# francescoolivieri/Gymnast_OptimalControl

Hardware: AMD Instinct MI355X
Metric: swing-up Newton iterations/sec (batch×T states/s) at 1/2/4/8 MI355X (higher is better)
Workload: dtype f64

## Files before the change

gymnast_optimalcontrol_amd/_lib.py:

```python
from __future__ import annotations

import ctypes as C
import os

import torch

from . import _build

LIB_PATH = os.environ.get("GYM_LIB_PATH") or _build.LIB_PATH

EXPORTS = (
    "gym_abi_version", "gym_build_id", "gym_model_from_params",
    "gym_continuous_dynamics", "gym_rk4_step", "gym_jacobians", "gym_stage_cost_derivs",
    "gym_pack_lanes", "gym_unpack_lanes", "gym_unpack_gains",
    "gym_rollout_open_loop", "gym_closed_loop", "gym_total_cost", "gym_backward_sweep", "gym_linearize",
    "gym_riccati_general",
    "gym_newton_init", "gym_newton_init_warm", "gym_newton_iteration", "gym_newton_pipeline_split", "gym_newton_phase", "gym_newton_phase_kind",
    "gym_newton_run",
    "gym_newton_tail", "gym_newton_tail_scratch", "gym_newton_cand_scratch", "gym_newton_tail_lds",
    "gym_newton_finalize", "gym_newton_fill_states", "gym_placement_probe", "gym_newton_sigma",
    "gym_gamma_sweep", "gym_newton_gamma_sweep",
    "gym_tv_lqr_gains", "gym_dare_fixed_point", "gym_mpc_gains", "gym_lq_forward", "gym_track_rollout", "gym_track_rollout_ex",
    "gym_mpc_gains_all", "gym_mpc_box_workspace", "gym_mpc_box_qp", "gym_mpc_box_rollout",
    "gym_lqr_lanes_workspace", "gym_lqr_lanes_gains", "gym_lqr_lanes_rollout",
    "gym_mpc_lanes_gains",
    "gym_mpc_box_lanes_workspace", "gym_mpc_box_lanes_rollout",
    "gym_timing_create", "gym_timing_destroy", "gym_timing_collect",
)
KERNEL_KINDS = ("backward", "trial", "candidates", "retry", "stats", "phase_odd", "phase_even", "sigma", "run",
                "tail")

ABI_VERSION = 18
MAX_BP = 1 << 26
MPC_MAX_STAGES = 256
FLAG_U0_ZERO = 1
FLAG_X_CKPT = 2
FLAG_RUN_SINGLE = 4
FLAG_REF_LANE = 8
FLAG_SIGMA_STREAM = 16
TRACK_SINGLE = 1
CKPT_INTERVAL = 4

ACTIVE, CONVERGED, LS_FAILED, MAX_ITERS, PAD = 0, 1, 2, 3, 4
STATUS_NAMES = {ACTIVE: "active", CONVERGED: "converged", LS_FAILED: "ls_failed", MAX_ITERS: "max_iters", PAD: "pad"}


class GymModel(C.Structure):
    _fields_ = [(n, C.c_double) for n in ("a", "b", "d", "g1", "g2", "f1", "f2", "dt")]


class GymWeights(C.Structure):
    _fields_ = [("Q", C.c_double * 4), ("R", C.c_double * 2), ("QT", C.c_double * 4)]


class GymArmijo(C.Structure):
    _fields_ = [("tol", C.c_double), ("beta", C.c_double), ("c", C.c_double), ("gamma0", C.c_double),
                ("max_ls", C.c_int32), ("record_history", C.c_int32)]


_P = C.c_void_p


TIMING_POOL = 512


class GymTiming(C.Structure):
    _fields_ = [("ev", _P * 20), ("ms", C.c_double * 10), ("launches", C.c_int64 * 10), ("pending", C.c_int32),
                ("pool_used", C.c_int32), ("pool_ev", _P * (2 * TIMING_POOL)), ("pool_kind", C.c_int32 * TIMING_POOL)]


class GymBatch(C.Structure):
    _fields_ = [("B", C.c_int64), ("Bp", C.c_int64), ("N", C.c_int32), ("hist_len", C.c_int32),
                ("flags", C.c_int32), ("pad", C.c_int32), ("x", _P * 2), ("u", _P * 2), ("K1", _P), ("cs", _P), ("x_ref", _P), ("u_ref", _P),
                ("cost", _P), ("dJ", _P), ("smax", _P), ("gamma", _P), ("status", _P), ("n_iter", _P),
                ("res_buf", _P), ("n_roll", _P), ("retry_list", _P), ("counters", _P), ("cand_ok", _P),
                ("partials", _P), ("stats", _P), ("hist_cost", _P), ("hist_smax", _P), ("lane_map", _P),
                ("timing", C.POINTER(GymTiming)), ("cand_scratch", _P), ("cand_slots", C.c_int64)]


_I64, _I32, _D = C.c_int64, C.c_int32, C.c_double
_MP, _WP, _AP, _BP = C.POINTER(GymModel), C.POINTER(GymWeights), C.POINTER(GymArmijo), C.POINTER(GymBatch)
_SIGS = {
    "gym_abi_version": [],
    "gym_model_from_params": [_P, _D, _MP],
    "gym_continuous_dynamics": [_MP, _P, _P, _P, _I64, _P],
    "gym_rk4_step": [_MP, _P, _P, _P, _I64, _P],
    "gym_jacobians": [_MP, _P, _P, _P, _P, _I64, _P],
    "gym_stage_cost_derivs": [_P, _P, _P, _P, _P, _P, _I32, _P, _P, _P, _I64, _P],
    "gym_pack_lanes": [_P, _P, _I64, _I64, _I32, _I32, _I32, _P],
    "gym_unpack_lanes": [_P, _P, _P, _P, _I64, _I64, _I32, _I32, _I32, _P],
    "gym_unpack_gains": [_P, _P, _I64, _I64, _I32, _P],
    "gym_rollout_open_loop": [_MP, _WP, _P, _P, _P, _P, _P, _P, _I64, _I64, _I32, _P],
    "gym_closed_loop": [_MP, _WP, _P, _P, _P, _P, _P, _P, _P, _P, _P, _P, _I64, _I64, _I32, _P],
    "gym_total_cost": [_P, _P, _P, _P, _P, _P, _P, _P, _I64, _I64, _I32, _P],
    "gym_backward_sweep": [_MP, _WP, _P, _P, _P, _P, _P, _P, _P, _P, _P, _I64, _I64, _I32, _P],
    "gym_linearize": [_MP, _WP, _P, _P, _P, _P, _P, _P, _P, _P, _P, _I64, _I64, _I32, _P],
    "gym_riccati_general": [_P] * 12 + [_I64, _I64, _I32, _P],
    "gym_newton_init": [_MP, _WP, _P, _BP, _P],
    "gym_newton_init_warm": [_MP, _WP, _P, _P, _P, _BP, _P],
    "gym_newton_iteration": [_MP, _WP, _AP, _BP, _I32, _P],
    "gym_newton_pipeline_split": [_BP, C.POINTER(C.c_int64)],
    "gym_newton_phase_kind": [_BP, C.POINTER(C.c_int32)],
    "gym_newton_phase": [_MP, _WP, _AP, _BP, _I32, _I32, _P],
    "gym_newton_run": [_MP, _WP, _AP, _BP, _I32, _I32, _P],
    "gym_newton_tail": [_MP, _WP, _AP, _BP, _P, _I32, _P, _I64, _I32, _I32, _P],
    "gym_newton_tail_scratch": [_I32, _I32, _I32, C.POINTER(C.c_int64)],
    "gym_newton_cand_scratch": [_I32, _I64, C.POINTER(C.c_int64)],
    "gym_newton_tail_lds": [_I32, C.POINTER(C.c_int64), C.POINTER(C.c_int64)],
    "gym_newton_finalize": [_MP, _WP, _BP, _I32, _P, _P, _P, _P, _P],
    "gym_newton_fill_states": [_MP, _BP, _I32, _P],
    "gym_placement_probe": [_BP, _I32, _P],
    "gym_newton_sigma": [_MP, _WP, _BP, _P, _P],
    "gym_gamma_sweep": [_MP, _WP, _P, _P, _P, _P, _P, _I32, _P, _P, _P, _I64, _I64, _I32, _P],
    "gym_newton_gamma_sweep": [_MP, _WP, _AP, _BP, _I32, _P, _I32, _P, _P],
    "gym_tv_lqr_gains": [_P, _P, _I32, _P, _P, _P, _P, _P, _I32, _I32, _I32, _I32, _D, _P, _P],
    "gym_dare_fixed_point": [_P, _P, _P, _P, _I32, _D, _P, _P, _P],
    "gym_mpc_gains": [_MP, _P, _P, _I32, _P, _P, _P, _P, _I32, _I32, _I32, _D, _P, _P, _P, _P],
    "gym_lq_forward": [_P, _P, _I32, _P, _P, _I32, _D, _P, _P, _I32, _P, _P, _P],
    "gym_track_rollout": [_MP, _P, _P, _P, _P, _I64, _I32, _P, _P, _P],
    "gym_track_rollout_ex": [_MP, _P, _P, _P, _P, _I64, _I32, _I32, _P, _P, _P],
    "gym_mpc_gains_all": [_MP, _P, _P, _I32, _P, _P, _P, _P, _I32, _I32, _I32, _D, _P, _P, _P, _P],
    "gym_mpc_box_workspace": [_I64, _I32, _I32, C.POINTER(C.c_int64)],
    "gym_mpc_box_qp": [_P, _P, _P, _I32, _P, _P, _P, _P, _I64, _I32, _D, _I32, _P, _I64, _P, _P, _P, _P, _P],
    "gym_mpc_box_rollout": [_MP, _P, _P, _P, _P, _P, _P, _P, _P, _P, _I64, _I32, _I32, _D, _I32, _P, _I64, _P, _P, _P,
                            _P, _P],
    "gym_lqr_lanes_workspace": [_I64, _I32, C.POINTER(C.c_int64)],
    "gym_lqr_lanes_gains": [_MP, _P, _P, _I64, _I32, _P, _P, _P, _P, _I64, _P, _P],
    "gym_lqr_lanes_rollout": [_MP, _P, _I64, _I32, _I32, _P, _I64, _P, _P, _P, _P],
    "gym_mpc_lanes_gains": [_MP, _P, _P, _I64, _I32, _I32, _P, _P, _P, _P, _I64, _P, _P],
    "gym_mpc_box_lanes_workspace": [_I64, _I32, _I32, C.POINTER(C.c_int64)],
    "gym_mpc_box_lanes_rollout": [_MP, _P, _P, _P, _I64, _I32, _I32, _I32, _P, _P, _P, _D, _I32, _P, _I64, _P, _P, _P,
                                  _P, _P, _P],
    "gym_timing_create": [C.POINTER(GymTiming)],
    "gym_timing_destroy": [C.POINTER(GymTiming)],
    "gym_timing_collect": [C.POINTER(GymTiming)],
}
# ... 52 lines not shown
```

gymnast_optimalcontrol_amd/csrc/acrobot_kernels.hip:

```cpp
#include <hip/hip_runtime.h>

#include <cstddef>
#include <cstdint>
#include <type_traits>

#include "acrobot_device.hpp"
#include "gymnast_acrobot.h"

using gym::Dyn;

namespace {

#include "newton_streams.hpp"
#include "newton_stages.hpp"
#include "newton_lockstep.hpp"
#include "newton_run.hpp"
#include "newton_tail.hpp"
#include "newton_util.hpp"

inline KW kw(const gym_weights& w) {
    KW k;
    for (int i = 0; i < 4; ++i) { k.Q[i] = w.Q[i]; k.QT[i] = w.QT[i]; k.twoQ[i] = 2.0 * w.Q[i]; }
    k.R[0] = w.R[0]; k.R[1] = w.R[1];
    k.G00 = 2.0 * w.R[0]; k.twoR1 = 2.0 * w.R[1]; k.iG00 = 1.0 / k.G00;
// ... 450 lines not shown
}

int gym_newton_init_warm(const gym_model* m, const gym_weights* w, const double* x0, const double* u_init,
                         const int32_t* status_init, const gym_batch* b, void* s) {
    if (!m || !w || !x0 || !u_init || bad_batch(b) || ((uintptr_t)u_init & 15)) return GYM_EINVAL;
    hipStream_t st = (hipStream_t)s;
    const int T = b->N - 1;
    if ((T + GP_TS - 1) / GP_TS > 65535) return GYM_EINVAL;
    const hipError_t e = reset_batch(b, false, st);
    if (e != hipSuccess) return (int)e;
    hipLaunchKernelGGL(k_gather_pack_u, dim3((unsigned)(b->Bp / BLK), (unsigned)((T + GP_TS - 1) / GP_TS)),
                       dim3(TILE_THREADS), 0, st, (const double2*)u_init, b->u[0], b->lane_map, b->B, b->Bp, T);
    int rc = launch_status();
    if (rc) return rc;
    hipLaunchKernelGGL(with_variant2(b, [](auto U0Z, auto RL) { return k_init_warm<U0Z(), RL()>; }),
                       dim3(grid_for(b->Bp, BLK)), dim3(BLK), 0, st, Dyn(*m), kw(*w), x0,
                       status_init, b->lane_map, b->u[0], b->x_ref, b->u_ref, (double2*)b->x[0], b->cost, b->status,
                       b->n_iter, b->res_buf, b->n_roll, b->gamma, b->smax, b->dJ, b->B, b->Bp, b->N);
    return launch_status();
}

constexpr int64_t POST_CAP = 2048;
constexpr int64_t CAND_CAP = 4096;
static CandScratch cand_scratch(const gym_batch* b, bool pair) {
    CandScratch c{nullptr, nullptr, nullptr, 0};
    if (!pair || !b->cand_scratch || b->cand_slots <= 0 || (b->flags & GYM_FLAG_X_CKPT)) return c;
    const int64_t V = b->cand_slots, N = b->N;
    c.sx = (double2*)b->cand_scratch;
    c.su = b->cand_scratch + 4 * N * V;
    c.sJ = c.su + 2 * (N - 1) * V;
    c.V = V;
    return c;
}
static void launch_post_trial(const gym_model* m, const gym_weights* w, const gym_armijo* a, const gym_batch* b,
                              const SolverCtl& c, const TrialIO& io, Range rg, int32_t* counter, double* stats_out,
                              const double* other, double* total, hipStream_t st, bool sigma_streamed = false) {
    const int64_t n = rg.hi - rg.lo;
    const double2* K1 = (const double2*)b->K1;
    const double* cs = b->cs;
    double* hc = a->record_history ? b->hist_cost : nullptr;
    if (a->max_ls > 1 && n > 0) {
        if (!sigma_streamed) {
            TimedLaunch tl(b->timing, 7, st);
            hipLaunchKernelGGL(sigma_kernel(b), dim3(grid_for(n, BLK, POST_CAP)), dim3(BLK), 0, st, Dyn(*m), kw(*w),
                               io.x, io.u, b->x_ref, b->u_ref, b->cs, b->retry_list + rg.lo, counter,
                               (const int32_t*)nullptr, -1, b->B, b->Bp, b->N);
        }
        const bool pair = !(b->flags & GYM_FLAG_RUN_SINGLE);
        const CandScratch sc = cand_scratch(b, pair);
        const int64_t ncand = n * (int64_t)(a->max_ls - 1);
        {
            TimedLaunch tl(b->timing, 2, st);
            if (pair)
                hipLaunchKernelGGL(with_variant2(b, [](auto U0Z, auto RL) { return k_nt_cand_pair<U0Z(), RL()>; }),
                                   dim3(grid_for(2 * ncand, BLK, CAND_CAP)), dim3(BLK), 0, st, Dyn(*m), kw(*w), c, io,
                                   K1, cs, b->x_ref, b->u_ref, b->cost, b->dJ, b->retry_list + rg.lo, counter,
                                   b->cand_ok, sc, b->Bp, b->N);
            else
                hipLaunchKernelGGL(with_variant2(b, [](auto U0Z, auto RL) { return k_nt_candidates<U0Z(), RL()>; }),
                                   dim3(grid_for(ncand, BLK, CAND_CAP)), dim3(BLK), 0, st, Dyn(*m), kw(*w), c, io, K1,
                                   cs, b->x_ref, b->u_ref, b->cost, b->dJ, b->retry_list + rg.lo, counter, b->cand_ok,
                                   b->Bp, b->N);
        }
        const int64_t items = sc.V > 0 ? n * (1 + (b->N + CPK - 1) / CPK) : n;
        TimedLaunch tl(b->timing, 3, st);
        hipLaunchKernelGGL(with_variant(b, [](auto U0Z, auto CK, auto RL) { return k_nt_retry<U0Z(), CK(), RL()>; }),
                           dim3(grid_for(items, BLK, POST_CAP)), dim3(BLK), 0, st, Dyn(*m), kw(*w), c, io, K1, cs,
                           b->x_ref, b->u_ref, b->cost, b->smax, b->gamma, b->status, b->n_iter, b->res_buf, b->n_roll,
                           b->retry_list + rg.lo, counter, b->cand_ok, hc, sc, b->Bp, b->N);
    }
    TimedLaunch tl(b->timing, 4, st);
    launch_stats(b, rg, c.k, counter, stats_out, other, total, st);
}

static TrialIO trial_io(const gym_batch* b, int k) {
    return TrialIO{(const double2*)b->x[k & 1], b->u[k & 1], (double2*)b->x[(k + 1) & 1], b->u[(k + 1) & 1]};
}

static bool bad_iter_args(const gym_model* m, const gym_weights* w, const gym_armijo* a, const gym_batch* b) {
    return !m || !w || !a || bad_batch(b) || a->max_ls < 1 || (a->max_ls > 1 && !b->cand_ok);
}

int gym_newton_iteration(const gym_model* m, const gym_weights* w, const gym_armijo* a, const gym_batch* b, int32_t k,
                         void* s) {
    if (bad_iter_args(m, w, a, b) || k < 0) return GYM_EINVAL;
    hipStream_t st = (hipStream_t)s;
    const Range all{0, b->B};
    const TrialIO io = trial_io(b, k);
    const int grid = grid_for(b->B, BLK);
    const bool hist = a->record_history != 0;
    const bool sig = (b->flags & GYM_FLAG_SIGMA_STREAM) != 0;
    {
        TimedLaunch tl(b->timing, 0, st);
        const auto sweep =
            with_variant(b, [](auto U0Z, auto CK, auto RL) { return k_nt_backward<U0Z(), CK(), RL()>; });
        hipLaunchKernelGGL(sig ? backward_all_kernel(b) : sweep, dim3(grid), dim3(BLK), 0, st, Dyn(*m), kw(*w), io.x,
                           io.u, b->x_ref, b->u_ref, (double2*)b->K1, b->cs, a->gamma0, b->dJ, b->smax, b->status,
                           hist ? b->hist_smax : nullptr, all, b->Bp, b->N, k, b->hist_len);
    }
    const SolverCtl c = solver_ctl(a, b, k);
    {
        TimedLaunch tl(b->timing, 1, st);
        hipLaunchKernelGGL(with_variant(b, [](auto U0Z, auto CK, auto RL) { return k_nt_trial<U0Z(), CK(), RL()>; }),
                           dim3(grid), dim3(BLK), 0, st, Dyn(*m), kw(*w), c, io, (const double2*)b->K1,
                           (const double*)b->cs, b->x_ref, b->u_ref, b->cost, b->dJ, b->smax, b->gamma, b->status,
                           b->n_iter, b->res_buf, b->n_roll, b->retry_list, b->counters, hist ? b->hist_cost : nullptr,
                           all, b->Bp, b->N);
    }
    launch_post_trial(m, w, a, b, c, io, all, b->counters, b->stats, nullptr, nullptr, st, sig);
    return launch_status();
}

static int device_cus() {
    static int cache[64] = {0};
    int dev = 0;
    if (hipGetDevice(&dev) != hipSuccess || dev < 0 || dev >= 64) return 0;
    if (!cache[dev]) {
        int n = 0;
        if (hipDeviceGetAttribute(&n, hipDeviceAttributeMultiprocessorCount, dev) == hipSuccess) cache[dev] = n;
    }
    return cache[dev];
}

constexpr int LO_MIN_EIGHTHS = 14;
static bool phase_low_occupancy(const gym_batch* b, int64_t waves) {
    if (b->flags & GYM_FLAG_X_CKPT) return false;
    const int64_t simds = 4 * (int64_t)device_cus();
    return simds > 0 && 8 * waves > LO_MIN_EIGHTHS * simds && waves <= 2 * simds;
}

int gym_newton_phase_kind(const gym_batch* b, int32_t* low_out) {
    if (bad_batch(b) || !low_out) return GYM_EINVAL;
    int64_t Bh;
    gym_newton_pipeline_split(b, &Bh);
    const int64_t waves = (Bh + BLK - 1) / BLK + (b->B - Bh + BLK - 1) / BLK;
    *low_out = phase_low_occupancy(b, waves) ? 1 : 0;
    return 0;
}

int gym_newton_pipeline_split(const gym_batch* b, int64_t* Bh) {
    if (!b || !Bh || b->B <= 0) return GYM_EINVAL;
    int64_t h = ((b->B + 1) / 2 + 63) / 64 * 64;
    *Bh = h < b->B ? h : b->B;
    return 0;
}

int gym_newton_phase(const gym_model* m, const gym_weights* w, const gym_armijo* a, const gym_batch* b, int32_t p,
                     int32_t do_backward, void* s) {
    if (bad_iter_args(m, w, a, b) || p < 0) return GYM_EINVAL;
    hipStream_t st = (hipStream_t)s;
    int64_t Bh;
    gym_newton_pipeline_split(b, &Bh);
    const Range half[2] = {{0, Bh}, {Bh, b->B}};
    const int hb = p & 1, kb = p >> 1;
    const Range rb = do_backward ? half[hb] : Range{0, 0};
    const int ht = (p & 1) ? 0 : 1;
    const int kt = (p & 1) ? (p - 1) >> 1 : (p - 2) >> 1;
    const Range rt = (p >= 1) ? half[ht] : Range{0, 0};
    const int nb_b = (int)((rb.hi - rb.lo + BLK - 1) / BLK), nb_t = (int)((rt.hi - rt.lo + BLK - 1) / BLK);
    const SolverCtl c = solver_ctl(a, b, kt < 0 ? 0 : kt);
    const TrialIO io = trial_io(b, c.k);
    if (nb_b + nb_t > 0) {
        TimedLaunch tl(b->timing, (p & 1) ? 5 : 6, st);
        PhaseArgs pa;
        shared_args(pa, m, w, a, b, c.k);
        pa.io = io;
        pa.xb_in = (const double2*)b->x[kb & 1]; pa.ub_in = b->u[kb & 1];
        pa.retry_list = b->retry_list; pa.counter = b->counters + ht;
        pa.rb = rb; pa.rt = rt; pa.Bp = b->Bp; pa.N = b->N; pa.kb = kb; pa.nb_b = nb_b; pa.pad = 0;
        hipLaunchKernelGGL(with_variant_no_ck(b, phase_low_occupancy(b, nb_b + nb_t),
                                              [](auto U0Z, auto CK, auto RL, auto LO) {
                                                  return k_nt_phase<U0Z(), CK(), RL(), LO()>;
                                              }),
                           dim3(nb_b + nb_t), dim3(BLK), 0, st, pa);
    }
    if (p >= 1)
        launch_post_trial(m, w, a, b, c, io, rt, b->counters + ht, b->stats + 8 + 8 * ht,
                          ht ? b->stats + 8 : nullptr, ht ? b->stats : nullptr, st);
    return launch_status();
}

int gym_newton_run(const gym_model* m, const gym_weights* w, const gym_armijo* a, const gym_batch* b, int32_t k0,
                   int32_t k1, void* s) {
    const bool ext = (b->flags & GYM_FLAG_SIGMA_STREAM) && !(b->flags & GYM_FLAG_RUN_SINGLE);
    if (bad_iter_args(m, w, a, b) || k0 < 0 || k1 < k0 || (b->flags & GYM_FLAG_X_CKPT) || (ext && k1 > k0 + 1))
        return GYM_EINVAL;
    hipStream_t st = (hipStream_t)s;
    const Range all{0, b->B};
    if (k1 > k0) {
        TimedLaunch tl(b->timing, 8, st);
        RunArgs ra;
        lane_args(ra, m, w, a, b, k0);
        ra.retry_list = b->retry_list; ra.counter = b->counters;
        ra.B = b->B; ra.Bp = b->Bp; ra.N = b->N; ra.k0 = k0; ra.k1 = k1; ra.ext = ext ? 1 : 0;
        if (b->flags & GYM_FLAG_RUN_SINGLE)
            hipLaunchKernelGGL(with_variant2(b, [](auto U0Z, auto RL) { return k_nt_run<U0Z(), RL()>; }),
                               dim3(grid_for(b->B, BLK)), dim3(BLK), 0, st, ra);
        else
            hipLaunchKernelGGL(with_variant2(b, [](auto U0Z, auto RL) { return k_nt_run2<U0Z(), RL()>; }),
                               dim3((unsigned)(b->Bp / BLK)), dim3(R2WAVES * BLK), 0, st, ra);
        if (ext) {
            launch_post_trial(m, w, a, b, ra.a, trial_io(b, k0), all, b->counters, b->stats, nullptr, nullptr, st, true);
            return launch_status();
        }
    }
    launch_stats(b, all, (int)k1 - 1, b->counters, b->stats, nullptr, nullptr, st);
    return launch_status();
}

int gym_newton_tail_scratch(int32_t N, int32_t n_lanes, int32_t max_ls, int64_t* doubles_out) {
    if (!doubles_out || N < 2 || N - 1 > TL_MAX_T || n_lanes < 0 || max_ls < 1 || max_ls > BLK) return GYM_EINVAL;
// ... 233 lines not shown
```

gymnast_optimalcontrol_amd/csrc/newton_lockstep.hpp:

```cpp
#pragma once

#ifdef GYM_WAVE_TRACE
__device__ unsigned long long g_wave_trace[2][8192][4];
struct WaveTrace {
    int kind;
    unsigned long long t0;
    __device__ explicit WaveTrace(int k) : kind(k), t0(__builtin_amdgcn_s_memrealtime()) {}
    __device__ ~WaveTrace() {
        if (threadIdx.x == 0 && blockIdx.x < 8192) {
            unsigned long long* r = g_wave_trace[kind][blockIdx.x];
            r[0] = t0;
            r[1] = __builtin_amdgcn_s_memrealtime();
            r[2] = (unsigned)__builtin_amdgcn_s_getreg((31 << 11) | 4);
            r[3] = (unsigned)__builtin_amdgcn_s_getreg((31 << 11) | 20);
        }
    }
};
#define GYM_TRACE_WAVE(k) WaveTrace wave_trace_(k)
#else
#define GYM_TRACE_WAVE(k)
#endif

constexpr int ck_lds_doubles(bool ck, bool u0z) { return ck ? (4 + (u0z ? 1 : 2)) * CKI * BLK : 2; }
#define GYM_CK_LDS(CK, U0Z) __shared__ double2 ck_lds[ck_lds_doubles(CK, U0Z) / 2]
// ... 337 lines not shown
                    if (t < N) {
                        io.xn[wix(t, 0, 2, l, Bp)] = sc.sx[wix(t, 0, 2, v, sc.V)];
                        io.xn[wix(t, 1, 2, l, Bp)] = sc.sx[wix(t, 1, 2, v, sc.V)];
                    }
                    if (t < T) {
                        if (!U0Z) io.un[pix(t, 0, 2, l, Bp)] = sc.su[pix(t, 0, 2, v, sc.V)];
                        io.un[pix(t, 1, 2, l, Bp)] = sc.su[pix(t, 1, 2, v, sc.V)];
                    }
                }
            }
            continue;
        }
        n_iter[l] += 1;
        if (jacc == 0) {
            n_roll[l] += nj;
            fail_lane(a, l, status, res_buf);
            continue;
        }
        n_roll[l] += jacc;
        double g = a.gamma0;
        for (int q = 0; q < jacc; ++q) g *= a.beta;
        double Jn;
        if (copy) {
            Jn = sc.sJ[v];
        } else {
            const double2 xa = io.x[wix(0, 0, 2, l, Bp)], xb = io.x[wix(0, 1, 2, l, Bp)];
            Jn = rollout_cform<true, U0Z, true, CK>(m, w, io.u, K1, cs, lane_ref<RL>(xr, l, 4 * (int64_t)N),
                                                    lane_ref<RL>(ur, l, 2 * (int64_t)(N - 1)), io.xn, io.un, g,
                                                    a.gamma0, l, Bp, N, xa.x, xa.y, xb.x, xb.y);
        }
        accept_lane(a, l, Jn, g, smax[l], cost, gamma, status, res_buf, hist_cost, Bp);
    }
}
```

gymnast_optimalcontrol_amd/solver.py:

```python
from __future__ import annotations

import ctypes as C
import time
import weakref
from collections import OrderedDict
from dataclasses import dataclass, field

import numpy as np
import torch

from . import _lib
from .engine import AcrobotEngine, padded, F64
from .params import DT, MAX_LINE_SEARCH_ITERS

STAT_FIELDS = ("n_active", "sum_cost", "sum_smax2", "lanes_ran", "n_retry", "n_converged", "n_failed", "n_rollouts")


@dataclass
class SolveResult:
    x: torch.Tensor
    u: torch.Tensor
    K: torch.Tensor
    sigma: torch.Tensor
    cost: torch.Tensor
# ... 230 lines not shown
        b = _lib.GymBatch()
        b.B, b.Bp, b.N, b.hist_len = self.B, self.Bp, self.N, self.hist_len
        ref_u0_zero = bool((self.u_ref[..., 0] == 0).all().item())
        if u0_zero and not ref_u0_zero:
            raise ValueError("u0_zero=True requires u_ref[:, 0] == 0")
        self.u0_zero = ref_u0_zero if u0_zero is None else bool(u0_zero)
        self._u0_cleared = False
        self.checkpoint = bool(checkpoint)
        if persistent and self.checkpoint:
            raise ValueError("the persistent schedule does not support state checkpointing")
        if persistent is None:
            persistent = pipeline is None and sched_B <= self.persistent_max_lanes(dev)
        self.persistent = bool(persistent) and not self.checkpoint
        self.chunk = int(chunk)
        self.reorder = bool(reorder)
        self.lane_order = None
        self.split_waves = bool(split_waves)
        b.flags = ((_lib.FLAG_U0_ZERO if self.u0_zero else 0) | (_lib.FLAG_X_CKPT if self.checkpoint else 0) |
                   (0 if self.split_waves else _lib.FLAG_RUN_SINGLE) | (_lib.FLAG_REF_LANE if self.ref_lane else 0))
        for name in ("cost", "dJ", "smax", "gamma", "status", "n_iter", "res_buf", "n_roll",
                     "retry_list", "counters", "cand_ok", "partials", "stats"):
            setattr(b, name, getattr(self, name).data_ptr())
        if self.ref_lane:
            b.x_ref, b.u_ref = self.xr_buf.data_ptr(), self.ur_buf.data_ptr()
        else:
            b.x_ref, b.u_ref = self.x_ref.data_ptr(), self.u_ref.data_ptr()
        b.hist_cost = _lib.ptr(self.hist_cost)
        b.hist_smax = _lib.ptr(self.hist_smax)
        self.batch = b
        self._set_streams(st)
        self.k = 0
        self.timeline = None
        self.timing = None
        self.launches = {"phase": 0, "run": 0, "tail": 0, "iteration": 0}
        self.capture_lanes = None if capture_lanes is None else [int(i) for i in capture_lanes]
        if self.capture_lanes is not None:
            if self.checkpoint:
                raise ValueError("trajectory capture needs the full state store (checkpoint=False)")
            if any(not (0 <= i < self.B) for i in self.capture_lanes):
                raise ValueError(f"capture_lanes must lie in [0, {self.B})")
        self.capture_every = max(int(capture_every), 1)
        self.capture_sigma = tuple(sorted({int(i) for i in (capture_sigma or ())}))
        self.tail_lanes_rank = None
        if tail_lanes is None:
            per_rank = (self.TAIL_LANES_PER_CU * torch.cuda.get_device_properties(dev).multi_processor_count
                        if auto_schedule else 0)
            tail_lanes = per_rank * max(int(world_size), 1)
            self.tail_lanes_rank = per_rank or None
        need, lds, lds_max = C.c_int64(), C.c_int64(), C.c_int64()
        tail_ok = (not self.persistent and not self.checkpoint and self.capture_lanes is None and
                   engine.lib.gym_newton_tail_scratch(self.N, 1, int(max_ls), C.byref(need)) == 0 and
                   engine.lib.gym_newton_tail_lds(self.N, C.byref(lds), C.byref(lds_max)) == 0 and
                   lds.value <= lds_max.value)
        self.tail_lanes = int(tail_lanes) if tail_ok else 0
        self.tail_chunk = max(int(tail_chunk), 1)
        if compact is None:
            compact = auto_schedule
        self.compact_mode = ("force" if compact == "force" else bool(compact)) if (
            not self.persistent and not self.checkpoint and self.capture_lanes is None) else False
        self.compactions = 0
        self._compact_prev = None
        self.lane_order_live = False
        self._serial_now = False
        self._run_now = False
        self.serial_switch_at = None
        self._its_switch, self._its_tail_start = 0, None
        self._tail_scratch = None
# ... 139 lines not shown
        st, rec = self._streams(), {k: v for k, v in self.placement.items() if k != "reused"}
        f = weakref.finalize(self, PlacementPool.put, self._pool_key, st, rec)
        f.atexit = False

    def ensure_cand_scratch(self) -> bool:
        if self._cand_scratch is None and self.cand_slots > 0:
            need = C.c_int64()
            _lib.check(self.eng.lib.gym_newton_cand_scratch(self.N, self.cand_slots, C.byref(need)),
                       "gym_newton_cand_scratch")
            self._cand_scratch = torch.empty(int(need.value), dtype=F64, device=self.eng.device)
            self.batch.cand_scratch, self.batch.cand_slots = self._cand_scratch.data_ptr(), self.cand_slots
        return self._cand_scratch is not None

    @property
    def schedule(self) -> str:
        return "persistent" if self.persistent else ("pipelined" if self.pipeline else "serial")

    def phase_kind(self) -> str | None:
        if self.schedule != "pipelined":
            return None
        lo = C.c_int32()
        _lib.check(self.eng.lib.gym_newton_phase_kind(C.byref(self.batch), C.byref(lo)), "gym_newton_phase_kind")
        return "two-wavefront" if lo.value else "four-wavefront"

    def enable_timing(self):
        if self.timing is None:
            t = _lib.GymTiming()
            _lib.check(self.eng.lib.gym_timing_create(C.byref(t)), "gym_timing_create")
            self.timing = t
            self.batch.timing = C.pointer(t)
        return self

    def reset_timing(self):
        self.launches = {"phase": 0, "run": 0, "tail": 0, "iteration": 0}
        if self.timing is not None:
            torch.cuda.synchronize(self.eng.device)
            self.collect_timing()
            for i in range(len(_lib.KERNEL_KINDS)):
                self.timing.ms[i] = 0.0
                self.timing.launches[i] = 0
            self.timing.pending = 0

    def collect_timing(self):
        if self.timing is not None:
            _lib.check(self.eng.lib.gym_timing_collect(C.byref(self.timing)), "gym_timing_collect")

    def kernel_times(self) -> dict:
        if self.timing is None:
            return {}
        return {k: (float(self.timing.ms[i]), int(self.timing.launches[i])) for i, k in enumerate(_lib.KERNEL_KINDS)}

    def __del__(self):
        t = getattr(self, "timing", None)
        if t is not None:
            try:
                self.eng.lib.gym_timing_destroy(C.byref(t))
            except Exception:
                pass

    def _warm_inputs(self, u_init, status_init):
        if isinstance(u_init, torch.Tensor) and u_init.dtype != F64:
            raise ValueError(f"u_init must be float64, got {u_init.dtype}")
        u = self.eng.t(u_init)
        if tuple(u.shape) != (self.B, self.T, 2):
            raise ValueError(f"u_init must be ({self.B},{self.T},2), got {tuple(u.shape)}")
        if u.data_ptr() % 16:
            u = u.clone()
# ... 21 lines not shown

    def init(self, x0, u_init=None, status_init=None, _ref_perm=None, _lane_map=None):
        self.lane_order = None
        self._restore_u0_zero()
        x0 = self.eng.t(x0).reshape(-1, 4)
        if x0.shape[0] != self.B:
            raise ValueError(f"x0 must hold {self.B} lanes, got {x0.shape[0]}")
        if u_init is None and status_init is not None:
            raise ValueError("status_init needs u_init (a lane's status belongs to its control iterate)")
        if u_init is not None:
            u_init, status_init = self._warm_inputs(u_init, status_init)
        if self.ref_lane:
            self.xr_buf[:self.B] = self._xr_in if _ref_perm is None else self._xr_in[_ref_perm]
            self.ur_buf[:self.B] = self._ur_in if _ref_perm is None else self._ur_in[_ref_perm]
        self._x0 = x0
        if self._pl is not None:
            self._placement_start()
        if u_init is None:
            _lib.check(self.eng.lib.gym_newton_init(C.byref(self.eng.model), C.byref(self.eng._w), x0.data_ptr(),
                                                    C.byref(self.batch), self.eng.stream), "gym_newton_init")
        else:
            if self.u0_zero and bool((u_init[..., 0] != 0).any().item()):
                self._set_u0_zero(False)
                self._u0_cleared = True
            self.batch.lane_map = None if _lane_map is None else _lane_map.data_ptr()
            try:
                _lib.check(self.eng.lib.gym_newton_init_warm(C.byref(self.eng.model), C.byref(self.eng._w),
                                                             x0.data_ptr(), u_init.data_ptr(), _lib.ptr(status_init),
                                                             C.byref(self.batch), self.eng.stream),
                           "gym_newton_init_warm")
            finally:
                self.batch.lane_map = None
        self.k = 0
        self._capture_start(self.capture_lanes or [])
        self._serial_now = False
        self._run_now = False
        self._sigma_streamed = False
        self.batch.flags &= ~_lib.FLAG_SIGMA_STREAM
        if self.pipeline and not self.persistent and (self.max_iters is None or self.max_iters > 0):
            self._phase(0, True)

    def _run(self, k0: int, k1: int):
        self.launches["run"] += 1
        _lib.check(self.eng.lib.gym_newton_run(C.byref(self.eng.model), C.byref(self.eng._w), C.byref(self.armijo),
                                               C.byref(self.batch), int(k0), int(k1), self.eng.stream),
                   "gym_newton_run")

    def tail_run(self, k0: int, k1: int) -> torch.Tensor:
        lanes = (self.status[:self.B] == _lib.ACTIVE).nonzero().flatten().to(torch.int32)
        n = int(lanes.numel())
        need = C.c_int64()
        _lib.check(self.eng.lib.gym_newton_tail_scratch(self.N, n, int(self.armijo.max_ls), C.byref(need)),
                   "gym_newton_tail_scratch")
        self.ensure_cand_scratch()
        if self._cand_scratch is not None and self._cand_scratch.numel() >= need.value:
            sc = self._cand_scratch
        else:
            if self._tail_scratch is None or self._tail_scratch.numel() < need.value:
                self._tail_scratch = None
                self._tail_scratch = torch.empty(int(need.value), dtype=F64, device=self.eng.device)
            sc = self._tail_scratch
        self.launches["tail"] += 1
        _lib.check(self.eng.lib.gym_newton_tail(C.byref(self.eng.model), C.byref(self.eng._w), C.byref(self.armijo),
                                                C.byref(self.batch), lanes.data_ptr() if n else None, n,
                                                sc.data_ptr(), int(sc.numel()), int(k0), int(k1), self.eng.stream),
                   "gym_newton_tail")
        self.k = int(k1)
        return self.stats[:8]

    def _phase(self, p: int, do_backward: bool):
        self.launches["phase"] += 1
        _lib.check(self.eng.lib.gym_newton_phase(C.byref(self.eng.model), C.byref(self.eng._w), C.byref(self.armijo),
                                                 C.byref(self.batch), p, int(do_backward), self.eng.stream),
                   "gym_newton_phase")

    def iteration(self) -> torch.Tensor:
        if self._pl is not None:
            self._placement_tick()
        k = self.k
        if self.persistent or self._run_now:
            self._run(k, k + 1)
        elif self.pipeline and not self._serial_now:
            more = self.max_iters is None or k + 1 < self.max_iters
            self._phase(2 * k + 1, True)
            self._phase(2 * k + 2, more)
        else:
            self.launches["iteration"] += 1
            _lib.check(self.eng.lib.gym_newton_iteration(C.byref(self.eng.model), C.byref(self.eng._w),
                                                         C.byref(self.armijo), C.byref(self.batch), k,
                                                         self.eng.stream), "gym_newton_iteration")
        self.k += 1
        self._capture()
        return self.stats[:8]

    def _capture_start(self, positions):
        self._cap_log = []
        self._sig_log = []
        if self.capture_lanes is None:
            self._cap_pos = None
            return
        self._cap_pos = torch.as_tensor(positions, dtype=torch.int64, device=self.eng.device)
        self._capture(initial=True)

    def _capture(self, initial: bool = False):
        if self._cap_pos is None or (not initial and self.k % self.capture_every):
            return
        pos = self._cap_pos
        W = self.Bp // 64
        xb = self.x[self.k & 1]
        x = xb.view(self.N, W, 2, 64, 2)[:, pos // 64, :, pos % 64, :].reshape(-1, self.N, 4)
        self._cap_log.append((self.k, x.clone(), self.n_iter[pos].clone(), self.status[pos].clone(),
                              self.cost[pos].clone()))
        if not initial and (self.k - 1) in self.capture_sigma:
            self._sig_log.append((self.k - 1, self.sigma()[pos].clone(), self.n_iter[pos].clone()))

    def captured_trajectories(self) -> dict:
        if self.capture_lanes is None:
            return {}
        out = {lane: [] for lane in self.capture_lanes}
        for k, x, n_it, st, _ in self._cap_log:
            x, n_it, st = x.cpu().numpy(), n_it.cpu().numpy(), st.cpu().numpy()
            for j, lane in enumerate(self.capture_lanes):
                if k == 0:
# ... 279 lines not shown
        if keep_stats:
            log.append(host.copy())
        if log_every:
            print(f"iter {k}: active={int(host[0])} sumJ={host[1]:.6e} ran={int(host[3])}", flush=True)
        if host[0] == 0:
            break
    return log


def newton_loop(stepper, max_iters: int, reduce_stats=None, sync_every: int = 1, log_every: int = 0,
                keep_stats: bool = False) -> list:
    log = []
    tail = int(getattr(stepper, "tail_lanes", 0) or 0)
    compact = getattr(stepper, "maybe_compact", None) if getattr(stepper, "lane_order_live", False) else None
    for k in range(int(max_iters)):
        st = stepper.iteration()
        if (k + 1) % sync_every == 0 or k + 1 == max_iters:
            local = st
            if reduce_stats is not None:
                st = reduce_stats(st)
            host = st.cpu().numpy() if isinstance(st, torch.Tensor) else np.asarray(st)
            collect = getattr(stepper, "collect_timing", None)
            if collect is not None:
                collect()
            if keep_stats:
                log.append(host.copy())
            if getattr(stepper, "timeline", None) is not None:
                stepper.timeline.append((k + 1, int(host[0]), time.perf_counter()))
            if log_every and (k % log_every == 0):
                print(f"iter {k}: active={int(host[0])} sumJ={host[1]:.6e} ran={int(host[3])} "
                      f"retry={int(host[4])}", flush=True)
            if host[0] == 0:
                break
            if host[4] > 0:
                ensure = getattr(stepper, "ensure_cand_scratch", None)
                if ensure is not None:
                    ensure()
            if tail and host[0] <= tail and k + 1 < max_iters and _tail_rank_ok(stepper, host, local, reduce_stats):
                log += tail_loop(stepper, k + 1, int(max_iters), reduce_stats, log_every, keep_stats)
                break
            if compact is not None and k + 1 < max_iters:
                compact(int(local[0].item()) if reduce_stats is not None else int(host[0]))
    return log


def _tail_rank_ok(stepper, host, local, reduce_stats) -> bool:
    cap = getattr(stepper, "tail_lanes_rank", None)
    if cap is None:
        return True
    if reduce_stats is None:
        return host[0] <= cap
    max_of = getattr(reduce_stats, "max_of", None)
    if max_of is None:
        if not getattr(stepper, "_warned_no_max_of", False):
            import warnings
            warnings.warn("reduce_stats has no max_of: the straggler tail's per-rank budget is not applied")
            stepper._warned_no_max_of = True
        return True
    n = float(local[0].item()) if isinstance(local, torch.Tensor) else float(np.asarray(local)[0])
    return max_of(n) <= cap


def tail_loop(solver, k: int, max_iters: int, reduce_stats, log_every: int, keep_stats: bool) -> list:
    log = []
    k_switch = k
    its0 = int(solver.n_iter[:solver.B].sum().item())
# ... 35 lines not shown
```

include/gymnast_acrobot.h:

```cpp
#ifndef GYMNAST_ACROBOT_H
#define GYMNAST_ACROBOT_H

#include <stdint.h>

#ifdef __cplusplus
extern "C" {
#endif

#define GYM_ABI_VERSION 18
#define GYM_MAX_BP (1LL << 26)

#define GYM_FLAG_U0_ZERO 1
#define GYM_FLAG_X_CKPT 2
#define GYM_FLAG_RUN_SINGLE 4
#define GYM_FLAG_REF_LANE 8
#define GYM_FLAG_SIGMA_STREAM 16
#define GYM_CKPT_INTERVAL 4
#define GYM_EINVAL 1

enum {
    GYM_ACTIVE = 0,
    GYM_CONVERGED = 1,
    GYM_LS_FAILED = 2,
    GYM_MAX_ITERS = 3,
// ... 70 lines not shown

int gym_pack_lanes(const double* src, double* dst, int64_t B, int64_t Bp, int32_t L, int32_t C, int32_t W,
                   void* stream);
int gym_unpack_lanes(const double* src0, const double* src1, const int32_t* sel, double* dst, int64_t B, int64_t Bp,
                     int32_t L, int32_t C, int32_t W, void* stream);
int gym_unpack_gains(const double* K1, double* K, int64_t B, int64_t Bp, int32_t T, void* stream);

int gym_rollout_open_loop(const gym_model* m, const gym_weights* w, const double* x0, const double* u,
                          const double* x_ref, const double* u_ref, double* x, double* cost, int64_t B, int64_t Bp,
                          int32_t N, void* stream);
int gym_closed_loop(const gym_model* m, const gym_weights* w, const double* x, const double* u, const double* Kf,
                    const double* sigma, const double* gamma, const double* x_ref, const double* u_ref,
                    double* x_new, double* u_new, double* cost, int64_t B, int64_t Bp, int32_t N, void* stream);
int gym_total_cost(const double* x, const double* u, const double* x_ref, const double* u_ref, const double Q[16],
                   const double R[4], const double QT[16], double* cost, int64_t B, int64_t Bp, int32_t N, void* stream);
int gym_backward_sweep(const gym_model* m, const gym_weights* w, const double* x, const double* u,
                       const double* x_ref, const double* u_ref, double* K1, double* sigma, double* dJ, double* smax,
                       double* lambda, int64_t B, int64_t Bp, int32_t N, void* stream);
int gym_linearize(const gym_model* m, const gym_weights* w, const double* x, const double* u, const double* x_ref,
                  const double* u_ref, double* A_d, double* B_d, double* q, double* r, double* qT, int64_t B,
                  int64_t Bp, int32_t N, void* stream);
int gym_riccati_general(const double* A, const double* Bm, const double* Q, const double* R, const double* S,
                        const double* q, const double* r, const double* QT, const double* qT, double* K, double* sigma,
                        double* dJ, int64_t B, int64_t Bp, int32_t T, void* stream);

int gym_newton_init(const gym_model* m, const gym_weights* w, const double* x0, const gym_batch* bt, void* stream);
int gym_newton_init_warm(const gym_model* m, const gym_weights* w, const double* x0, const double* u_init,
                         const int32_t* status_init, const gym_batch* bt, void* stream);
int gym_newton_iteration(const gym_model* m, const gym_weights* w, const gym_armijo* a, const gym_batch* bt,
                         int32_t k, void* stream);
int gym_newton_pipeline_split(const gym_batch* bt, int64_t* Bh);
int gym_newton_phase(const gym_model* m, const gym_weights* w, const gym_armijo* a, const gym_batch* bt, int32_t p,
                     int32_t do_backward, void* stream);
int gym_newton_phase_kind(const gym_batch* bt, int32_t* low_out);
int gym_newton_run(const gym_model* m, const gym_weights* w, const gym_armijo* a, const gym_batch* bt, int32_t k0,
                   int32_t k1, void* stream);
int gym_newton_tail(const gym_model* m, const gym_weights* w, const gym_armijo* a, const gym_batch* bt,
                    const int32_t* lanes, int32_t n_lanes, double* scratch, int64_t scratch_doubles, int32_t k0,
                    int32_t k1, void* stream);
int gym_newton_tail_scratch(int32_t N, int32_t n_lanes, int32_t max_ls, int64_t* doubles_out);
int gym_newton_cand_scratch(int32_t N, int64_t slots, int64_t* doubles_out);
int gym_newton_tail_lds(int32_t N, int64_t* bytes_out, int64_t* limit_out);
int gym_newton_finalize(const gym_model* m, const gym_weights* w, const gym_batch* bt, int32_t k_done, double* x_out,
                        double* u_out, double* K_out, double* sigma_out, void* stream);
int gym_newton_fill_states(const gym_model* m, const gym_batch* bt, int32_t buf, void* stream);
int gym_placement_probe(const gym_batch* bt, int32_t cb, void* stream);
int gym_newton_sigma(const gym_model* m, const gym_weights* w, const gym_batch* bt, double* sigma_out, void* stream);

int gym_gamma_sweep(const gym_model* m, const gym_weights* w, const double* x, const double* u, const double* Kf,
                    const double* sigma, const double* gammas, int32_t G, const double* x_ref, const double* u_ref,
                    double* cost_out, int64_t B, int64_t Bp, int32_t N, void* stream);
int gym_newton_gamma_sweep(const gym_model* m, const gym_weights* w, const gym_armijo* a, const gym_batch* bt,
                           int32_t k, const double* gammas, int32_t G, double* cost_out, void* stream);

int gym_tv_lqr_gains(const double* A, const double* B, int32_t S, const double* A_pad, const double* B_pad,
                     const double Q[16], const double R[4], const double QT[16], int32_t L, int32_t nwin,
                     int32_t all_gains, int32_t discretize, double dt, double* K_out, void* stream);
int gym_dare_fixed_point(const double* A, const double* B, const double Q[16], const double R[4], int32_t max_iter,
                         double tol, double* P_out, int32_t* iters_out, void* stream);
int gym_mpc_gains(const gym_model* m, const double* x_ref, const double* u_ref, int32_t S, const double* x_f,
                  const double* u_f, const double Q[16], const double R[4], int32_t L, int32_t nwin, int32_t max_iter,
                  double tol, double* K_out, double* QT_out, int32_t* iters_out, void* stream);
int gym_lq_forward(const double* A, const double* B, int32_t S, const double* A_pad, const double* B_pad,
                   int32_t discretize, double dt, const double* K, const double* x0, int32_t L, double* X, double* U,
                   void* stream);
int gym_track_rollout(const gym_model* m, const double* x0, const double* x_ff, const double* u_ff, const double* K,
// ... 47 lines not shown
```

Before: 63.72 million.

## Fuse post-trial sigma, candidate and retry kernels into one launch when retries vanish

Adds a fused k_nt_post kernel. Each block handles one retry lane and runs that lane's backward sigma solve, its paired-thread candidate rollouts and the accept/copy step, separated by block barriers. The host picks this path only when the previous iteration reported zero retries, so a likely-empty post-trial stage costs one small launch instead of several. When retries do occur, the per-lane backward solve runs on a single thread per block, which could serialize work compared with the separate kernels.

```diff
diff --git a/gymnast_optimalcontrol_amd/_lib.py b/gymnast_optimalcontrol_amd/_lib.py
--- a/gymnast_optimalcontrol_amd/_lib.py
+++ b/gymnast_optimalcontrol_amd/_lib.py
@@ -15,7 +15,8 @@
     "gym_pack_lanes", "gym_unpack_lanes", "gym_unpack_gains",
     "gym_rollout_open_loop", "gym_closed_loop", "gym_total_cost", "gym_backward_sweep", "gym_linearize",
     "gym_riccati_general",
-    "gym_newton_init", "gym_newton_init_warm", "gym_newton_iteration", "gym_newton_pipeline_split", "gym_newton_phase", "gym_newton_phase_kind",
+    "gym_newton_init", "gym_newton_init_warm", "gym_newton_iteration", "gym_newton_pipeline_split", "gym_newton_phase",
+    "gym_newton_iteration_opt", "gym_newton_phase_opt", "gym_newton_phase_kind",
     "gym_newton_run",
     "gym_newton_tail", "gym_newton_tail_scratch", "gym_newton_cand_scratch", "gym_newton_tail_lds",
     "gym_newton_finalize", "gym_newton_fill_states", "gym_placement_probe", "gym_newton_sigma",
@@ -40,6 +41,7 @@
 FLAG_SIGMA_STREAM = 16
 TRACK_SINGLE = 1
 CKPT_INTERVAL = 4
+OPT_POST_EMPTY = 1
 
 ACTIVE, CONVERGED, LS_FAILED, MAX_ITERS, PAD = 0, 1, 2, 3, 4
 STATUS_NAMES = {ACTIVE: "active", CONVERGED: "converged", LS_FAILED: "ls_failed", MAX_ITERS: "max_iters", PAD: "pad"}
@@ -102,6 +104,8 @@
     "gym_newton_pipeline_split": [_BP, C.POINTER(C.c_int64)],
     "gym_newton_phase_kind": [_BP, C.POINTER(C.c_int32)],
     "gym_newton_phase": [_MP, _WP, _AP, _BP, _I32, _I32, _P],
+    "gym_newton_iteration_opt": [_MP, _WP, _AP, _BP, _I32, _I32, _P],
+    "gym_newton_phase_opt": [_MP, _WP, _AP, _BP, _I32, _I32, _I32, _P],
     "gym_newton_run": [_MP, _WP, _AP, _BP, _I32, _I32, _P],
     "gym_newton_tail": [_MP, _WP, _AP, _BP, _P, _I32, _P, _I64, _I32, _I32, _P],
     "gym_newton_tail_scratch": [_I32, _I32, _I32, C.POINTER(C.c_int64)],
diff --git a/gymnast_optimalcontrol_amd/csrc/acrobot_kernels.hip b/gymnast_optimalcontrol_amd/csrc/acrobot_kernels.hip
--- a/gymnast_optimalcontrol_amd/csrc/acrobot_kernels.hip
+++ b/gymnast_optimalcontrol_amd/csrc/acrobot_kernels.hip
@@ -506,14 +506,24 @@
     c.V = V;
     return c;
 }
+constexpr int64_t FUSED_CAP = 256;
 static void launch_post_trial(const gym_model* m, const gym_weights* w, const gym_armijo* a, const gym_batch* b,
                               const SolverCtl& c, const TrialIO& io, Range rg, int32_t* counter, double* stats_out,
-                              const double* other, double* total, hipStream_t st, bool sigma_streamed = false) {
+                              const double* other, double* total, hipStream_t st, bool sigma_streamed = false,
+                              int opts = 0) {
     const int64_t n = rg.hi - rg.lo;
     const double2* K1 = (const double2*)b->K1;
     const double* cs = b->cs;
     double* hc = a->record_history ? b->hist_cost : nullptr;
-    if (a->max_ls > 1 && n > 0) {
+    const bool fused = (opts & GYM_OPT_POST_EMPTY) && !sigma_streamed && !(b->flags & GYM_FLAG_RUN_SINGLE);
+    if (a->max_ls > 1 && n > 0 && fused) {
+        TimedLaunch tl(b->timing, 3, st);
+        hipLaunchKernelGGL(with_variant(b, [](auto U0Z, auto CK, auto RL) { return k_nt_post<U0Z(), CK(), RL()>; }),
+                           dim3(grid_for(n, 1, FUSED_CAP)), dim3(BLK), 0, st, Dyn(*m), kw(*w), c, io, K1, b->cs,
+                           b->x_ref, b->u_ref, b->cost, b->dJ, b->smax, b->gamma, b->status, b->n_iter, b->res_buf,
+                           b->n_roll, b->retry_list + rg.lo, counter, b->cand_ok, hc, cand_scratch(b, true), b->Bp,
+                           b->N);
+    } else if (a->max_ls > 1 && n > 0) {
         if (!sigma_streamed) {
             TimedLaunch tl(b->timing, 7, st);
             hipLaunchKernelGGL(sigma_kernel(b), dim3(grid_for(n, BLK, POST_CAP)), dim3(BLK), 0, st, Dyn(*m), kw(*w),
@@ -557,7 +567,12 @@
 
 int gym_newton_iteration(const gym_model* m, const gym_weights* w, const gym_armijo* a, const gym_batch* b, int32_t k,
                          void* s) {
-    if (bad_iter_args(m, w, a, b) || k < 0) return GYM_EINVAL;
+    return gym_newton_iteration_opt(m, w, a, b, k, 0, s);
+}
+
+int gym_newton_iteration_opt(const gym_model* m, const gym_weights* w, const gym_armijo* a, const gym_batch* b,
+                             int32_t k, int32_t opts, void* s) {
+    if (bad_iter_args(m, w, a, b) || k < 0 || (opts & ~GYM_OPT_ALL)) return GYM_EINVAL;
     hipStream_t st = (hipStream_t)s;
     const Range all{0, b->B};
     const TrialIO io = trial_io(b, k);
@@ -581,7 +596,7 @@
                            b->n_iter, b->res_buf, b->n_roll, b->retry_list, b->counters, hist ? b->hist_cost : nullptr,
                            all, b->Bp, b->N);
     }
-    launch_post_trial(m, w, a, b, c, io, all, b->counters, b->stats, nullptr, nullptr, st, sig);
+    launch_post_trial(m, w, a, b, c, io, all, b->counters, b->stats, nullptr, nullptr, st, sig, opts);
     return launch_status();
 }
 
@@ -621,7 +636,12 @@
 
 int gym_newton_phase(const gym_model* m, const gym_weights* w, const gym_armijo* a, const gym_batch* b, int32_t p,
                      int32_t do_backward, void* s) {
-    if (bad_iter_args(m, w, a, b) || p < 0) return GYM_EINVAL;
+    return gym_newton_phase_opt(m, w, a, b, p, do_backward, 0, s);
+}
+
+int gym_newton_phase_opt(const gym_model* m, const gym_weights* w, const gym_armijo* a, const gym_batch* b, int32_t p,
+                         int32_t do_backward, int32_t opts, void* s) {
+    if (bad_iter_args(m, w, a, b) || p < 0 || (opts & ~GYM_OPT_ALL)) return GYM_EINVAL;
     hipStream_t st = (hipStream_t)s;
     int64_t Bh;
     gym_newton_pipeline_split(b, &Bh);
@@ -650,7 +670,7 @@
     }
     if (p >= 1)
         launch_post_trial(m, w, a, b, c, io, rt, b->counters + ht, b->stats + 8 + 8 * ht,
-                          ht ? b->stats + 8 : nullptr, ht ? b->stats : nullptr, st);
+                          ht ? b->stats + 8 : nullptr, ht ? b->stats : nullptr, st, false, opts);
     return launch_status();
 }
 
diff --git a/gymnast_optimalcontrol_amd/csrc/newton_lockstep.hpp b/gymnast_optimalcontrol_amd/csrc/newton_lockstep.hpp
--- a/gymnast_optimalcontrol_amd/csrc/newton_lockstep.hpp
+++ b/gymnast_optimalcontrol_amd/csrc/newton_lockstep.hpp
@@ -393,3 +393,180 @@
         accept_lane(a, l, Jn, g, smax[l], cost, gamma, status, res_buf, hist_cost, Bp);
     }
 }
+
+template <bool U0Z, bool RL>
+__device__ __forceinline__ void cand_pair_items(const Dyn& m, const KW& w, const SolverCtl& a, const TrialIO& io,
+                                                const double2* K1, const double* cs,
+                                                const double* xr, const double* ur,
+                                                const double* cost, const double* dJ,
+                                                const int32_t* retry_list,
+                                                uint8_t* cand_ok, const CandScratch& sc, int64_t Bp,
+                                                int N, int64_t first, int64_t end, int64_t stride) {
+    const int nj = a.max_ls - 1;
+    const int64_t total = end;
+    const int T = N - 1;
+    const bool odd = threadIdx.x & 1;
+    const uint32_t srow = (uint32_t)sc.V * 16u, splane = (uint32_t)sc.V * 8u;
+    const uint32_t row = (uint32_t)Bp * 16u, plane = (uint32_t)Bp * 8u;
+    const char* Kb = reinterpret_cast<const char*>(K1);
+    const char* Cb = reinterpret_cast<const char*>(cs);
+    const char* Ub = reinterpret_cast<const char*>(io.u);
+    const char* Xs = reinterpret_cast<const char*>(sc.sx);
+    const char* Us = reinterpret_cast<const char*>(sc.su);
+    const gym::PolyRegs pk = gym::poly_vgprs_all();
+    Dyn dm = m;
+    gym::in_vgpr(dm.b); gym::in_vgpr(dm.d); gym::in_vgpr(dm.a2b); gym::in_vgpr(dm.bb); gym::in_vgpr(dm.dad);
+    gym::in_vgpr(dm.g1); gym::in_vgpr(dm.g2); gym::in_vgpr(dm.f1); gym::in_vgpr(dm.f2); gym::in_vgpr(dm.h);
+    gym::in_vgpr(dm.h2); gym::in_vgpr(dm.h6);
+    for (int64_t base = first; base < total; base += stride) {
+        const int64_t i0 = base + (threadIdx.x >> 1);
+        const bool act = i0 < total;
+        const int64_t i = act ? i0 : total - 1;
+        const int64_t r = i / nj;
+        const int j = 1 + (int)(i % nj);
+        const int64_t l = retry_list[r];
+        double g = a.gamma0;
+        for (int q = 0; q < j; ++q) g *= a.beta;
+        const double dg = g - a.gamma0;
+        const bool keep = act && i < sc.V;
+        constexpr uint32_t OOB = 0x80000000u;
+        const uint32_t o2 = wbo(l, 2), o1 = (uint32_t)l * 8u;
+        const uint32_t v2 = keep ? wbo(i, 2) + (odd ? WROW : 0u) : OOB;
+        const uint32_t v1o = keep && !odd ? (uint32_t)i * 8u : OOB;
+        const double* xrl = lane_ref<RL>(xr, l, 4 * (int64_t)N);
+        const double* url = lane_ref<RL>(ur, l, 2 * (int64_t)T);
+        const double2 xa = io.x[wix(0, 0, 2, l, Bp)], xb = io.x[wix(0, 1, 2, l, Bp)];
+        double n0 = xa.x, n1 = xa.y, n2 = xb.x, n3 = xb.y;
+        bst2(rsrc(Xs), v2, 0, odd ? n2 : n0, odd ? n3 : n1);
+        auto fetch = [&](TrialStage& q, int t) {
+            const auto rK = rsrc(Kb + (int64_t)t * (2 * (int64_t)row));
+            q.k0 = bld2(rK, o2, 0);
+            q.k1 = bld2(rK, o2, WROW);
+            const auto rC = rsrc(Cb + (int64_t)t * row);
+            q.cg = bld1(rC, o1, 0);
+            q.s1 = bld1(rC, o1, plane);
+            q.u0 = U0Z ? 0.0 : bld1(rsrc(Ub + (int64_t)t * row), o1, 0);
+        };
+        const double G00 = w.G00, iG00 = w.iG00;
+        double J = 0.0;
+        TrialStage pre;
+        fetch(pre, 0);
+        for (int t = 0; t < T; ++t) {
+            const TrialStage q = pre;
+            if (t + 1 < T) fetch(pre, t + 1);
+            const double* urt = url + 2 * t;
+            const double v0 = U0Z ? 0.0 : trial_u0(q.u0, urt[0], g, G00, iG00);
+            const double v1 = trial_u1_sig(q.k0, q.k1, q.cg, q.s1, dg, n0, n1, n2, n3);
+            const double f0 = U0Z ? 0.0 : v0 - urt[0], f1 = v1 - urt[1];
+            J = stage_cost<U0Z>(J, w.Q, w.R, n0, n1, n2, n3, xrl + 4 * t, f0, f1);
+            {
+                const auto rO = rsrc(Us + (int64_t)t * srow);
+                if (!U0Z) bst1(rO, v1o, 0, v0);
+                bst1(rO, v1o, splane, v1);
+            }
+            gym::rk4_pair_fast<true>(dm, odd, n0, n1, n2, n3, v1, pk);
+            bst2(rsrc(Xs + (int64_t)(t + 1) * (2 * (int64_t)srow)), v2, 0, odd ? n2 : n0, odd ? n3 : n1);
+        }
+        const double Jn = J + xcost(w.QT, n0, n1, n2, n3, xrl + 4 * T);
+        if (act && !odd) {
+            cand_ok[(int64_t)j * Bp + l] = (Jn < cost[l] + a.c * g * dJ[l]) ? 1 : 0;
+            if (keep) sc.sJ[i] = Jn;
+        }
+    }
+}
+
+__device__ __forceinline__ int retry_copy_items(const CandScratch& sc, int N) {
+    return sc.V > 0 ? (N + CPK - 1) / CPK : 0;
+}
+template <bool U0Z, bool CK, bool RL>
+__device__ __forceinline__ void retry_item(const Dyn& m, const KW& w, const SolverCtl& a, const TrialIO& io,
+                                           const double2* K1, const double* cs,
+                                           const double* xr, const double* ur,
+                                           double* cost, const double* smax,
+                                           double* gamma, int32_t* status,
+                                           int32_t* n_iter, int32_t* res_buf,
+                                           int32_t* n_roll, const int32_t* retry_list,
+                                           const uint8_t* cand_ok, double* hist_cost,
+                                           const CandScratch& sc, int64_t Bp, int N, bool head, int64_t ri, int c) {
+    const int nj = a.max_ls - 1;
+    const int T = N - 1;
+    const int64_t l = retry_list[ri];
+    int jacc = 0;
+    for (int j0 = 1; j0 <= nj && jacc == 0; j0 += 8) {
+        uint8_t ok[8];
+#pragma unroll
+        for (int q = 0; q < 8; ++q) ok[q] = j0 + q <= nj ? cand_ok[(int64_t)(j0 + q) * Bp + l] : 0;
+#pragma unroll
+        for (int q = 7; q >= 0; --q)
+            if (ok[q]) jacc = j0 + q;
+    }
+    const int64_t v = ri * nj + jacc - 1;
+    const bool copy = jacc > 0 && v < sc.V;
+    if (!head) {
+        if (copy) {
+#pragma unroll
+            for (int q = 0; q < CPK; ++q) {
+                const int t = c * CPK + q;
+                if (t < N) {
+                    io.xn[wix(t, 0, 2, l, Bp)] = sc.sx[wix(t, 0, 2, v, sc.V)];
+                    io.xn[wix(t, 1, 2, l, Bp)] = sc.sx[wix(t, 1, 2, v, sc.V)];
+                }
+                if (t < T) {
+                    if (!U0Z) io.un[pix(t, 0, 2, l, Bp)] = sc.su[pix(t, 0, 2, v, sc.V)];
+                    io.un[pix(t, 1, 2, l, Bp)] = sc.su[pix(t, 1, 2, v, sc.V)];
+                }
+            }
+        }
+        return;
+    }
+    n_iter[l] += 1;
+    if (jacc == 0) {
+        n_roll[l] += nj;
+        fail_lane(a, l, status, res_buf);
+        return;
+    }
+    n_roll[l] += jacc;
+    double g = a.gamma0;
+    for (int q = 0; q < jacc; ++q) g *= a.beta;
+    double Jn;
+    if (copy) {
+        Jn = sc.sJ[v];
+    } else {
+        const double2 xa = io.x[wix(0, 0, 2, l, Bp)], xb = io.x[wix(0, 1, 2, l, Bp)];
+        Jn = rollout_cform<true, U0Z, true, CK>(m, w, io.u, K1, cs, lane_ref<RL>(xr, l, 4 * (int64_t)N),
+                                                lane_ref<RL>(ur, l, 2 * (int64_t)(N - 1)), io.xn, io.un, g,
+                                                a.gamma0, l, Bp, N, xa.x, xa.y, xb.x, xb.y);
+    }
+    accept_lane(a, l, Jn, g, smax[l], cost, gamma, status, res_buf, hist_cost, Bp);
+}
+
+template <bool U0Z, bool CK, bool RL = false>
+__global__ __launch_bounds__(BLK) void k_nt_post(Dyn m, KW w, SolverCtl a, TrialIO io, const double2* K1, double* cs,
+                                                 const double* __restrict__ xr, const double* __restrict__ ur,
+                                                 double* cost, const double* __restrict__ dJ,
+                                                 const double* __restrict__ smax, double* __restrict__ gamma,
+                                                 int32_t* status, int32_t* n_iter, int32_t* res_buf, int32_t* n_roll,
+                                                 const int32_t* __restrict__ retry_list,
+                                                 const int32_t* __restrict__ counter, uint8_t* cand_ok,
+                                                 double* __restrict__ hist_cost, CandScratch sc, int64_t Bp, int N) {
+    GYM_CK_LDS(CK, U0Z);
+    const int nr = *counter;
+    const int nj = a.max_ls - 1;
+    const int nc = retry_copy_items(sc, N);
+    for (int64_t r = blockIdx.x; r < nr; r += gridDim.x) {
+        if (threadIdx.x == 0) {
+            const int64_t l = retry_list[r];
+            backward_solver<U0Z, CK, OUT_SIGMA>(m, w, io.x, io.u, lane_ref<RL>(xr, l, 4 * (int64_t)N),
+                                                lane_ref<RL>(ur, l, 2 * (int64_t)(N - 1)), nullptr, cs, 0.0, nullptr,
+                                                nullptr, nullptr, l, Bp, N, 0, 0, ck_lds);
+        }
+        __syncthreads();
+        cand_pair_items<U0Z, RL>(m, w, a, io, K1, cs, xr, ur, cost, dJ, retry_list, cand_ok, sc, Bp, N, r * nj,
+                                 (r + 1) * nj, BLK / 2);
+        __syncthreads();
+        for (int it = threadIdx.x; it < 1 + nc; it += BLK)
+            retry_item<U0Z, CK, RL>(m, w, a, io, K1, cs, xr, ur, cost, smax, gamma, status, n_iter, res_buf, n_roll,
+                                    retry_list, cand_ok, hist_cost, sc, Bp, N, it == 0, r, it - 1);
+        __syncthreads();
+    }
+}
diff --git a/gymnast_optimalcontrol_amd/solver.py b/gymnast_optimalcontrol_amd/solver.py
--- a/gymnast_optimalcontrol_amd/solver.py
+++ b/gymnast_optimalcontrol_amd/solver.py
@@ -286,7 +286,9 @@
         self.k = 0
         self.timeline = None
         self.timing = None
-        self.launches = {"phase": 0, "run": 0, "tail": 0, "iteration": 0}
+        self.launches = {"phase": 0, "run": 0, "tail": 0, "iteration": 0, "post": 0}
+        self.launch_opts = None
+        self._retry_seen = None
         self.capture_lanes = None if capture_lanes is None else [int(i) for i in capture_lanes]
         if self.capture_lanes is not None:
             if self.checkpoint:
@@ -492,7 +494,7 @@
         return self
 
     def reset_timing(self):
-        self.launches = {"phase": 0, "run": 0, "tail": 0, "iteration": 0}
+        self.launches = {"phase": 0, "run": 0, "tail": 0, "iteration": 0, "post": 0}
         if self.timing is not None:
             torch.cuda.synchronize(self.eng.device)
             self.collect_timing()
@@ -580,6 +582,7 @@
             finally:
                 self.batch.lane_map = None
         self.k = 0
+        self._retry_seen = None
         self._capture_start(self.capture_lanes or [])
         self._serial_now = False
         self._run_now = False
@@ -616,11 +619,22 @@
         self.k = int(k1)
         return self.stats[:8]
 
+    def note_retry(self, n_retry: int):
+        self._retry_seen = int(n_retry)
+
+    def _opts(self, post_trial: bool = True) -> int:
+        opts = self.launch_opts
+        if opts is None:
+            opts = _lib.OPT_POST_EMPTY if self._retry_seen == 0 else 0
+        if post_trial and (opts & _lib.OPT_POST_EMPTY) and self.armijo.max_ls > 1 and self.split_waves:
+            self.launches["post"] += 1
+        return int(opts)
+
     def _phase(self, p: int, do_backward: bool):
         self.launches["phase"] += 1
-        _lib.check(self.eng.lib.gym_newton_phase(C.byref(self.eng.model), C.byref(self.eng._w), C.byref(self.armijo),
-                                                 C.byref(self.batch), p, int(do_backward), self.eng.stream),
-                   "gym_newton_phase")
+        _lib.check(self.eng.lib.gym_newton_phase_opt(C.byref(self.eng.model), C.byref(self.eng._w),
+                                                     C.byref(self.armijo), C.byref(self.batch), p, int(do_backward),
+                                                     self._opts(p >= 1), self.eng.stream), "gym_newton_phase_opt")
 
     def iteration(self) -> torch.Tensor:
         if self._pl is not None:
@@ -634,9 +648,9 @@
             self._phase(2 * k + 2, more)
         else:
             self.launches["iteration"] += 1
-            _lib.check(self.eng.lib.gym_newton_iteration(C.byref(self.eng.model), C.byref(self.eng._w),
-                                                         C.byref(self.armijo), C.byref(self.batch), k,
-                                                         self.eng.stream), "gym_newton_iteration")
+            _lib.check(self.eng.lib.gym_newton_iteration_opt(
+                C.byref(self.eng.model), C.byref(self.eng._w), C.byref(self.armijo), C.byref(self.batch), k,
+                self._opts(not self._sigma_streamed), self.eng.stream), "gym_newton_iteration_opt")
         self.k += 1
         self._capture()
         return self.stats[:8]
@@ -982,6 +996,9 @@
                       f"retry={int(host[4])}", flush=True)
             if host[0] == 0:
                 break
+            note = getattr(stepper, "note_retry", None)
+            if note is not None:
+                note(int(host[4]))
             if host[4] > 0:
                 ensure = getattr(stepper, "ensure_cand_scratch", None)
                 if ensure is not None:
diff --git a/include/gymnast_acrobot.h b/include/gymnast_acrobot.h
--- a/include/gymnast_acrobot.h
+++ b/include/gymnast_acrobot.h
@@ -126,6 +126,12 @@
 int gym_newton_pipeline_split(const gym_batch* bt, int64_t* Bh);
 int gym_newton_phase(const gym_model* m, const gym_weights* w, const gym_armijo* a, const gym_batch* bt, int32_t p,
                      int32_t do_backward, void* stream);
+#define GYM_OPT_POST_EMPTY 1
+#define GYM_OPT_ALL 1
+int gym_newton_iteration_opt(const gym_model* m, const gym_weights* w, const gym_armijo* a, const gym_batch* bt,
+                             int32_t k, int32_t opts, void* stream);
+int gym_newton_phase_opt(const gym_model* m, const gym_weights* w, const gym_armijo* a, const gym_batch* bt, int32_t p,
+                         int32_t do_backward, int32_t opts, void* stream);
 int gym_newton_phase_kind(const gym_batch* bt, int32_t* low_out);
 int gym_newton_run(const gym_model* m, const gym_weights* w, const gym_armijo* a, const gym_batch* bt, int32_t k0,
                    int32_t k1, void* stream);
```

Result: no change. 63.96 million (median of 6 runs) (+0.4%).
